# V-Sense/LFBM5D

Hardware: AMD Instinct MI355X
Metric: SAI-megapixels/sec (HT+Wiener, sigma=25) (higher is better)
Workload: dtype f32; 1 GPU; lf17x17x512x512_sigma25; light_field=17x17x512x512x3, asw=1, color_space=opp, noise=MT19937 seed 1 (utilities.cpp:176-183), window_lanes=2, spatial_bands=1, parallelism=single GPU

## Files before the change

### lfbm5d_amd/core.py

```python
import ctypes as C
import os
import subprocess

from typing import NamedTuple, Optional

import numpy as np

_HERE = os.path.dirname(os.path.abspath(__file__))

YUV, YCBCR, OPP, RGB, ID, DCT, SADCT, BIOR, HADAMARD, HAAR = range(10)
ROWMAJOR, COLMAJOR = 11, 12
TAU = {"id": ID, "dct": DCT, "sadct": SADCT, "bior": BIOR, "hw": HADAMARD, "haar": HAAR}
COLOR_SPACE = {"yuv": YUV, "ycbcr": YCBCR, "opp": OPP, "rgb": RGB}
UNIQUE_ID_BYTES = 128


class LfBm5dError(RuntimeError):
    pass


class Params(C.Structure):
    _fields_ = [("sigma", C.c_float), ("lambda_", C.c_float), ("N", C.c_uint), ("nSim", C.c_uint),
                ("nDisp", C.c_uint), ("k", C.c_uint), ("p", C.c_uint), ("useSD", C.c_uint),
                ("tau_2D", C.c_uint), ("tau_4D", C.c_uint), ("tau_5D", C.c_uint),
# ... 194 lines not shown
    dp = C.POINTER(C.c_double)
    if lib().lfbm5d_noise_level_statistic(d, cov.ctypes.data_as(dp), C.byref(sig), C.byref(m), lam.ctypes.data_as(dp)) != 0:
        raise LfBm5dError("lfbm5d_noise_level_statistic: bad arguments (d must be 1..64)")
    return sig.value, m.value, lam


def shard_rows(n_rows, rank, world):
    b, e = C.c_uint(), C.c_uint()
    lib().lfbm5d_shard_rows(n_rows, rank, world, C.byref(b), C.byref(e))
    return b.value, e.value


def make_params(sigma, lam, N, nSim, nDisp, k, p, tau_2D, tau_4D, tau_5D, useSD=0, color_space=OPP):
    t = lambda v: TAU[v] if isinstance(v, str) else int(v)
    cs = COLOR_SPACE[color_space] if isinstance(color_space, str) else int(color_space)
    return Params(float(sigma), float(lam), int(N), int(nSim), int(nDisp), int(k), int(p),
                  int(bool(useSD)), t(tau_2D), t(tau_4D), t(tau_5D), cs)


def make_bm3d_params(sigma, lam, N, nHW, k, p, tau_2D, useSD=0, color_space=OPP):
    cs = COLOR_SPACE[color_space] if isinstance(color_space, str) else int(color_space)
    return Bm3dParams(float(sigma), float(lam), int(N), int(nHW), int(k), int(p), int(bool(useSD)),
                      TAU[tau_2D] if isinstance(tau_2D, str) else int(tau_2D), cs)


def _u32(a):
    return np.ascontiguousarray(np.asarray(a, dtype=np.uint32))


def _dev_ptr(t):
    import torch
    if not (isinstance(t, torch.Tensor) and t.is_cuda and t.dtype == torch.float32 and t.is_contiguous()):
        raise LfBm5dError("device entry points need contiguous float32 CUDA tensors")
    torch.cuda.current_stream(t.device).synchronize()
    return C.c_void_p(t.data_ptr())


def _sai_ptrs(arrays, mask):
    out = (C.c_void_p * len(arrays))()
    for i, a in enumerate(arrays):
        if a is None or not mask[i]:
            continue
        if not (isinstance(a, np.ndarray) and a.dtype == np.float32 and a.flags.c_contiguous):
            raise LfBm5dError("per-SAI host buffers must be contiguous float32 numpy arrays")
        out[i] = a.ctypes.data
    return out


OPTION_ENV = ("LFBM5D_LANES", "LFBM5D_EMULATE_WORLD", "LFBM5D_MAX_WINDOWS", "LFBM5D_FUSED", "LFBM5D_STEP_SHARDING",
              "LFBM5D_DATA_DRIVEN_SCHEDULE", "LFBM5D_HOST_BLOCKING", "LFBM5D_BAND_MB", "LFBM5D_BM3D_LANES", "LFBM5D_SCAN_LDS_CAP",
              "LFBM5D_FORCE_REDO", "LFBM5D_SPATIAL_BANDS", "LFBM5D_BAND_HALO", "LFBM5D_SCAN_V1", "LFBM5D_SCAN_ANY", "LFBM5D_SCAN_FULL_TABLES", "LFBM5D_DCT8W_V2",
              "LFBM5D_GROUP_GENERIC", "LFBM5D_NO_SA_KERNELS", "LFBM5D_NO_SLAB_KERNEL", "LFBM5D_WIDE_NOSPLIT", "LFBM5D_AGG_64BIT",
              "LFBM5D_AGG_SCALAR_SCAN", "LFBM5D_SUBSET_LIST_HOST", "LFBM5D_SUBSET_SCAN_V1", "LFBM5D_FILT_GROUP_MAJOR",
              "LFBM5D_HT_REF_ORDER")


class Context:

    def __init__(self, device=0):
        self._L = lib()
        h = C.c_void_p()
        if self._L.lfbm5d_create(C.byref(h), int(device)) != 0:
            raise LfBm5dError(self._L.lfbm5d_last_error(None).decode())
        self._handle = h
        self._env_seen = {k: os.environ.get(k) for k in OPTION_ENV}
        self.device = int(device)

    @property
    def _h(self):
        h = self._handle
        if h and hasattr(self._L, "lfbm5d_set_option"):
            for k in OPTION_ENV:
                v = os.environ.get(k)
                if v != self._env_seen[k]:
                    self._env_seen[k] = v
                    self._L.lfbm5d_set_option(h, k.encode(), None if v is None else (v or "1").encode())
        return h

    def set_option(self, key, value):
        if self._L.lfbm5d_set_option(self._handle, key.encode(), None if value is None else str(value).encode()) != 0:
            raise LfBm5dError(self._L.lfbm5d_last_error(self._handle).decode())

    def get_option(self, key):
        buf = C.create_string_buffer(64)
        if self._L.lfbm5d_get_option(self._handle, key.encode(), buf, 64) != 0:
            raise LfBm5dError(self._L.lfbm5d_last_error(self._handle).decode())
        return buf.value.decode()

    def close(self):
        if getattr(self, "_handle", None):
            self._L.lfbm5d_destroy(self._handle)
            self._handle = None

    def __del__(self):
        try:
            self.close()
        except Exception:
            pass

    def _ck(self, rc):
        if rc != 0:
            raise LfBm5dError(self._L.lfbm5d_last_error(self._h).decode())

    @staticmethod
    def unique_id():
        buf = (C.c_ubyte * UNIQUE_ID_BYTES)()
        if lib().lfbm5d_comm_unique_id(buf) != 0:
# ... 237 lines not shown
```

### lfbm5d_amd/csrc/lfbm5d_group_wiener.hip

```cpp
#include "lfbm5d_group_device.h"

namespace lfbm5d {

namespace {

constexpr int kDct8Threads = 320;

__global__ __launch_bounds__(kDct8Threads) void k_group_dct8(GroupArgs a) {
    extern __shared__ float lds[];
    __shared__ unsigned pos[kMaxN * kA3];
    __shared__ float red[3][kDct8Threads / 64];
    const int tid = threadIdx.x;
    const unsigned g = a.ref_begin + blockIdx.x;
    const int c = blockIdx.y;
    constexpr int A = 9, K2 = 64;
    const int N = a.N;
    const int nSx = (int)a.self_cnt[g];
    const size_t plane = (size_t)a.Wb * a.Hb;
    const int NP = nSx * A;
    const int NPp = (N * A) | 1;
    float* S0 = lds;
    float* S1 = lds + K2 * NPp;
    const TbPtr tb = (TbPtr)a.tb;

// ... 719 lines not shown
            const float Nn = (float)(nSx * A);
            const float res = (q - m * m / Nn) / (Nn - 1.0f);
            wx = res > 0.0f ? 1.0f / sqrtf(res) : 0.0f;
        } else {
            const float sig = a.sigma[c];
            wx = w > 0.0f ? (sig > 0.0f ? 1.0f / (sig * sig * w) : 1.0f / w) : 1.0f;
        }
        a.wgt[(size_t)g * a.C + c] = wx;
        if (c == 0) {
            atomicAdd(&a.counters[0], (unsigned long long)nSx);
            if (use_sadct) atomicAdd(&a.counters[1], 1ull);
        }
    }

    PHASE_MARK();
    const int NPh = (NP + 1) / 2;
    for (int it = tid; it < NPh * 8; it += TH) {
        const int j = (int)__umulhi((unsigned)it, rcpNPh), pa = it - j * NPh;
        const int pb = pa + NPh < NP ? pa + NPh : pa;
        float* ca = stackf + 2 * (j * NPp + pa) + 1;
        float* cb = stackf + 2 * (j * NPp + pb) + 1;
        v2f x[8];
#pragma unroll
        for (int i = 0; i < 8; i++) x[i] = v2f{ca[2 * (i * 8) * NPp], cb[2 * (i * 8) * NPp]};
        dct8_inv_t(x);
#pragma unroll
        for (int i = 0; i < 8; i++) { ca[2 * (i * 8) * NPp] = x[i].x; if (pb != pa) cb[2 * (i * 8) * NPp] = x[i].y; }
    }
    __syncthreads();
    PHASE_MARK();
    for (int it = tid; it < NP * 8; it += TH) {
        const int patch = it >> 3, i = it & 7;
        const float* ra = stackf + 2 * ((i * 8) * NPp + patch) + 1;
        float x[8];
#pragma unroll
        for (int j = 0; j < 8; j++) x[j] = ra[2 * j * NPp];
        dct8_inv_t(x);
        float4* oa = reinterpret_cast<float4*>(a.filt + ((size_t)g * N * A + patch) * a.C * K2 + (size_t)c * K2 + i * 8);
        filt_put4(&oa[0], make_float4(x[0], x[1], x[2], x[3]));
        filt_put4(&oa[1], make_float4(x[4], x[5], x[6], x[7]));
    }
#ifdef LFBM5D_PHASE_TIMING
    PHASE_MARK();
    if (tid == 0) {
        for (int i = 0; i < 5; i++) atomicAdd(&a.counters[4 + i], (unsigned long long)(tc[i + 1] - tc[i]));
        atomicAdd(&a.counters[9], 1ull);
    }
#endif
}

constexpr int kDct8w3Threads = 256;
constexpr int kW3Stride = 146;
constexpr unsigned kW3Lds = 64 * kW3Stride * sizeof(float);
constexpr unsigned kW3Empty = 0xf0000000u;

template <int NS, int TH> struct W3Rows {
    static constexpr int kIt = (((NS * 9 + 1) / 2) * 8 + TH - 1) / TH;
    v4f ra0[kIt], ra1[kIt], rb0[kIt], rb1[kIt];
};
template <int NS, int TH>
__device__ __forceinline__ void w3_load_rows(__amdgpu_buffer_rsrc_t img, unsigned row_bytes, const unsigned* pos, int tid, W3Rows<NS, TH>& r) {
    constexpr int A = 9, NP = NS * A, NPh = (NP + 1) / 2;
#pragma unroll
    for (int q = 0; q < W3Rows<NS, TH>::kIt; q++) {
        const int it = tid + q * TH;
        if (it < NPh * 8) {
            const int i = it / NPh, pp = it - i * NPh;
            const int pA = 2 * pp, pB = pA + 1 < NP ? pA + 1 : pA;
            const int oa = (int)(pos[pA] + (unsigned)i * row_bytes), ob = (int)(pos[pB] + (unsigned)i * row_bytes);
            r.ra0[q] = __builtin_bit_cast(v4f, __builtin_amdgcn_raw_buffer_load_b128(img, oa, 0, 0));
            r.ra1[q] = __builtin_bit_cast(v4f, __builtin_amdgcn_raw_buffer_load_b128(img, oa + 16, 0, 0));
            r.rb0[q] = __builtin_bit_cast(v4f, __builtin_amdgcn_raw_buffer_load_b128(img, ob, 0, 0));
            r.rb1[q] = __builtin_bit_cast(v4f, __builtin_amdgcn_raw_buffer_load_b128(img, ob + 16, 0, 0));
        }
    }
}
template <int NS, int TH, bool SA, bool U = false>
__device__ __forceinline__ void w3_forward(__amdgpu_buffer_rsrc_t img, unsigned row_bytes, float* S, const unsigned* pos,
                                           int tid, ShRef sh, bool do_dct4, bool do_sa4, TbPtr tb, const W3Rows<NS, TH>* pre = nullptr) {
    constexpr int A = 9, NP = NS * A, NPh = (NP + 1) / 2, NPf = kW3Stride;
    constexpr int kIt = (NPh * 8 + TH - 1) / TH;
    {
        W3Rows<NS, TH> own;
        if (!pre) w3_load_rows<NS, TH>(img, row_bytes, pos, tid, own);
        const W3Rows<NS, TH>& R = pre ? *pre : own;
        const v4f (&ra0)[kIt] = R.ra0; const v4f (&ra1)[kIt] = R.ra1; const v4f (&rb0)[kIt] = R.rb0; const v4f (&rb1)[kIt] = R.rb1;
#pragma unroll
        for (int q = 0; q < kIt; q++) {
            const int it = tid + q * TH;
            if (it < NPh * 8) {
                const int i = it / NPh, pp = it - i * NPh;
                v2f x[8];
#pragma unroll
                for (int j = 0; j < 4; j++) {
                    x[j] = v2f{ra0[q][j], rb0[q][j]};
                    x[4 + j] = v2f{ra1[q][j], rb1[q][j]};
                }
                dct8_fwd_t(x);
                float* dst = S + (i * 8) * NPf + 2 * pp;
#pragma unroll
                for (int j = 0; j < 8; j++) *reinterpret_cast<v2f*>(dst + j * NPf) = x[j];
            }
        }
    }
    __syncthreads();
    for (int it = tid; it < NPh * 8; it += TH) {
        const int j = it / NPh, pp = it - j * NPh;
        float* col = S + j * NPf + 2 * pp;
        v2f x[8];
#pragma unroll
        for (int i = 0; i < 8; i++) x[i] = *reinterpret_cast<const v2f*>(col + (i * 8) * NPf);
        dct8_fwd_t(x);
#pragma unroll
        for (int i = 0; i < 8; i++) *reinterpret_cast<v2f*>(col + (i * 8) * NPf) = x[i];
    }
    __syncthreads();
    if (do_dct4 || do_sa4) {
        for (int f = tid; f < NS * 32; f += TH) {
            int n, pq;
            if (NS > 1) { pq = (f & 15) | ((f >> 1) & 16); n = ((f >> 4) & 1) | ((f >> 5) & ~1); }
            else { n = 0; pq = f; }
            float* b0 = S + pq * NPf + n * A;
            float* b1 = b0 + 32 * NPf;
            v2f x[9];
#pragma unroll
            for (int st = 0; st < 9; st++) x[st] = v2f{b0[st], b1[st]};
            if (U) dct9_fwd2_u(x);
            else if (do_dct4) dct9_fwd2_fast(x, tb);
            else {
                float t9[9];
#pragma unroll
                for (int i = 0; i < 9; i++) t9[i] = x[i].x;
                if (SA) sadct9_fwd_sel(t9, sh, tb); else sadct9_fwd(t9, sh, tb);
#pragma unroll
                for (int i = 0; i < 9; i++) { x[i].x = t9[i]; t9[i] = x[i].y; }
                if (SA) sadct9_fwd_sel(t9, sh, tb); else sadct9_fwd(t9, sh, tb);
#pragma unroll
                for (int i = 0; i < 9; i++) x[i].y = t9[i];
            }
#pragma unroll
            for (int st = 0; st < 9; st++) { b0[st] = x[st].x; b1[st] = x[st].y; }
        }
        __syncthreads();
    }
}

template <int NS, int TH, bool SA>
__device__ __forceinline__ void w3_body(const GroupArgs& a, float* S, const unsigned* pos, float (*red)[TH / 64], int tid,
                                        unsigned g, int c) {
    constexpr int A = 9, K2 = 64, NP = NS * A, NPh = (NP + 1) / 2, NPf = kW3Stride;
    static_assert(TH == 256, "the fibre phases deal st 0..3 / 4..7 to 256 threads");
    const int N = a.N;
    const unsigned win_bytes = (unsigned)((size_t)A * a.C * a.Wb * a.Hb * 4);
    const TbPtr tb = (TbPtr)a.tb;
    ShRef sh = group_shape(a, g);
    const bool use_sadct = a.tau4 == 6 && sh.use_sadct;
    const bool do_dct4 = a.tau4 == 5 || (a.tau4 == 6 && !use_sadct);
    const bool do_sa4 = !do_dct4 && a.tau4 == 6;
    const float sig = a.sigma[c];
    const float sig2 = sig * sig;
    const bool useSD = a.useSD != 0;

    w3_forward<NS, TH, SA>(__builtin_amdgcn_make_buffer_rsrc((void*)a.basic, 0, (int)win_bytes, 0x00020000u), a.Wb * 4u, S, pos, tid, sh, do_dct4, do_sa4, tb);
    const int fpq = (tid & 15) | ((tid >> 1) & 48), fst = ((tid >> 4) & 1) | ((tid >> 6) & 2);
    float* const fbase = S + fpq * NPf + fst;
    float* const f8base = S + (tid & 63) * NPf + 8;
    const bool own8 = tid < 64;
    v2f vv[NS];
    float v8[NS];
    {
        v2f e[NS];
// ... 102 lines not shown
            }
#pragma unroll
            for (int st = 0; st < 9; st++) { b0[st] = x[st].x; b1[st] = x[st].y; }
        }
    }
    __syncthreads();
    if (tid == 0) {
        float w = 0.0f, m = 0.0f, q = 0.0f;
        for (int i = 0; i < TH / 64; i++) { w += red[0][i]; m += red[1][i]; q += red[2][i]; }
        float wx;
        if (a.useSD) {
            const float Nn = (float)(NS * A);
            const float res = (q - m * m / Nn) / (Nn - 1.0f);
            wx = res > 0.0f ? 1.0f / sqrtf(res) : 0.0f;
        } else {
            wx = w > 0.0f ? (sig > 0.0f ? 1.0f / (sig * sig * w) : 1.0f / w) : 1.0f;
        }
        a.wgt[(size_t)g * a.C + c] = wx;
        if (c == 0) {
            atomicAdd(&a.counters[0], (unsigned long long)NS);
            if (use_sadct) atomicAdd(&a.counters[1], 1ull);
        }
    }
    for (int it = tid; it < NPh * 8; it += TH) {
        const int j = it / NPh, pp = it - j * NPh;
        float* col = S + j * NPf + 2 * pp;
        v2f x[8];
#pragma unroll
        for (int i = 0; i < 8; i++) x[i] = *reinterpret_cast<const v2f*>(col + (i * 8) * NPf);
        dct8_inv_t(x);
#pragma unroll
        for (int i = 0; i < 8; i++) *reinterpret_cast<v2f*>(col + (i * 8) * NPf) = x[i];
    }
    __syncthreads();
    for (int it = tid; it < NPh * 8; it += TH) {
        const int pa = it >> 3, i = it & 7;
        const bool has_b = pa + NPh < NP;
        const float* ra = S + (i * 8) * NPf + pa;
        v2f x[8];
#pragma unroll
        for (int j = 0; j < 8; j++) x[j] = v2f{ra[j * NPf], ra[j * NPf + (NP > NPh ? NPh : 0)]};
        dct8_inv_t(x);
        v4f* oa = reinterpret_cast<v4f*>(a.filt + ((size_t)g * N * A + pa) * a.C * K2 + (size_t)c * K2 + i * 8);
        filt_put4_nt(oa, v4f{x[0].x, x[1].x, x[2].x, x[3].x});
        filt_put4_nt(oa + 1, v4f{x[4].x, x[5].x, x[6].x, x[7].x});
        if (has_b) {
            v4f* ob = oa + (size_t)NPh * a.C * (K2 / 4);
            filt_put4_nt(ob, v4f{x[0].y, x[1].y, x[2].y, x[3].y});
            filt_put4_nt(ob + 1, v4f{x[4].y, x[5].y, x[6].y, x[7].y});
        }
    }
}

template <int NS, int TH>
__device__ __forceinline__ void w3_body_u(const GroupArgs& a, float* S, const unsigned* pos, float (*red)[TH / 64], int tid, unsigned g, int c) {
    constexpr int A = 9, K2 = 64, NP = NS * A, NPh = (NP + 1) / 2, NPf = kW3Stride;
    constexpr int L = NS == 16 ? 4 : NS == 8 ? 3 : NS == 4 ? 2 : NS == 2 ? 1 : 0;
    static_assert(TH == 256, "the fibre phases deal st 0..3 / 4..7 to 256 threads");
    const int N = a.N;
    const unsigned win_bytes = (unsigned)((size_t)A * a.C * a.Wb * a.Hb * 4);
    const TbPtr tb = (TbPtr)a.tb;
    ShRef sh = group_shape(a, g);
    const float sig = a.sigma[c];
    const float sig2 = sig * sig;
    const bool useSD = a.useSD != 0;

    w3_forward<NS, TH, false, true>(__builtin_amdgcn_make_buffer_rsrc((void*)a.basic, 0, (int)win_bytes, 0x00020000u), a.Wb * 4u, S, pos, tid, sh, true, false, tb);
    const int fpq = (tid & 15) | ((tid >> 1) & 48), fst = ((tid >> 4) & 1) | ((tid >> 6) & 2);
    float* const fbase = S + fpq * NPf + fst;
    float* const f8base = S + (tid & 63) * NPf + 8;
    const bool own8 = tid < 64;
    v2f kq[L + 1];
    float k8[L + 1];
    {
        const float fa = tb->ht3_f[fst], fb = tb->ht3_f[fst + 4], f8 = tb->ht3_f[8];
        const v2f q = v2f{sig2 / (fa * fa), sig2 / (fb * fb)};
        const float q8 = sig2 / (f8 * f8);
#pragma unroll
        for (int l = 0; l <= L; l++) { kq[l] = q * (float)(1 << l); k8[l] = q8 * (float)(1 << l); }
    }
    v2f vv[NS];
    float v8[NS];
    {
        v2f e[NS];
#pragma unroll
        for (int n = 0; n < NS; n++) e[n] = v2f{fbase[n * A], fbase[n * A + 4]};
        haar_fwd_u<NS>(e);
#pragma unroll
        for (int n = 0; n < NS; n++) {
            const v2f value = e[n] * e[n], den = value + kq[haar_level<NS>(n)];
            vv[n] = v2f{wiener_div(value.x, den.x), wiener_div(value.y, den.y)};
        }
    }
    if (own8) {
        float e[NS];
#pragma unroll
        for (int n = 0; n < NS; n++) e[n] = f8base[n * A];
        haar_fwd_u<NS>(e);
#pragma unroll
        for (int n = 0; n < NS; n++) {
            const float value = e[n] * e[n];
            v8[n] = wiener_div(value, value + k8[haar_level<NS>(n)]);
        }
    }
    __syncthreads();
    w3_forward<NS, TH, false, true>(__builtin_amdgcn_make_buffer_rsrc((void*)a.noisy, 0, (int)win_bytes, 0x00020000u), a.Wb * 4u, S, pos, tid, sh, true, false, tb);
    float wacc = 0.0f, s1 = 0.0f, s2 = 0.0f;
    const float inv_n = 1.0f / (float)NS;
    {
        v2f o[NS];
#pragma unroll
        for (int n = 0; n < NS; n++) o[n] = v2f{fbase[n * A], fbase[n * A + 4]};
        haar_fwd_u<NS>(o);
        v2f w2 = v2f{0.f, 0.f};
#pragma unroll
        for (int n = 0; n < NS; n++) { o[n] = o[n] * vv[n]; w2 += vv[n]; }
        wacc = w2.x + w2.y;
        haar_inv_u<NS>(o);
#pragma unroll
        for (int n = 0; n < NS; n++) { fbase[n * A] = o[n].x; fbase[n * A + 4] = o[n].y; }
        if (useSD) {
            const v2f f2 = v2f{tb->ht3_f[fst], tb->ht3_f[fst + 4]} * inv_n;
#pragma unroll
            for (int n = 0; n < NS; n++) { const v2f y = o[n] * f2; s1 += y.x + y.y; s2 += y.x * y.x + y.y * y.y; }
        }
    }
    if (own8) {
        float o[NS];
#pragma unroll
        for (int n = 0; n < NS; n++) o[n] = f8base[n * A];
        haar_fwd_u<NS>(o);
#pragma unroll
        for (int n = 0; n < NS; n++) { o[n] = o[n] * v8[n]; wacc += v8[n]; }
        haar_inv_u<NS>(o);
#pragma unroll
        for (int n = 0; n < NS; n++) f8base[n * A] = o[n];
        if (useSD) {
            const float f2 = tb->ht3_f[8] * inv_n;
#pragma unroll
            for (int n = 0; n < NS; n++) { const float y = o[n] * f2; s1 += y; s2 += y * y; }
        }
    }
    for (int o = 32; o > 0; o >>= 1) { wacc += __shfl_xor(wacc, o); s1 += __shfl_xor(s1, o); s2 += __shfl_xor(s2, o); }
    if ((tid & 63) == 0) { red[0][tid >> 6] = wacc; red[1][tid >> 6] = s1; red[2][tid >> 6] = s2; }
    __syncthreads();
    for (int f = tid; f < NS * 32; f += TH) {
        int n, pq;
        if (NS > 1) { pq = (f & 15) | ((f >> 1) & 16); n = ((f >> 4) & 1) | ((f >> 5) & ~1); }
        else { n = 0; pq = f; }
        float* b0 = S + pq * NPf + n * A;
        float* b1 = b0 + 32 * NPf;
        v2f x[9];
#pragma unroll
        for (int st = 0; st < 9; st++) x[st] = v2f{b0[st], b1[st]};
        dct9_inv2_u(x, tb, inv_n);
#pragma unroll
        for (int st = 0; st < 9; st++) { b0[st] = x[st].x; b1[st] = x[st].y; }
    }
    __syncthreads();
    if (tid == 0) {
        float w = 0.0f, m = 0.0f, q = 0.0f;
        for (int i = 0; i < TH / 64; i++) { w += red[0][i]; m += red[1][i]; q += red[2][i]; }
        float wx;
        if (a.useSD) {
            const float Nn = (float)(NS * A);
            const float res = (q - m * m / Nn) / (Nn - 1.0f);
            wx = res > 0.0f ? 1.0f / sqrtf(res) : 0.0f;
        } else {
            wx = w > 0.0f ? (sig > 0.0f ? 1.0f / (sig * sig * w) : 1.0f / w) : 1.0f;
        }
        a.wgt[(size_t)g * a.C + c] = wx;
        if (c == 0) atomicAdd(&a.counters[0], (unsigned long long)NS);
    }
    for (int it = tid; it < NPh * 8; it += TH) {
        const int j = it / NPh, pp = it - j * NPh;
        float* col = S + j * NPf + 2 * pp;
        v2f x[8];
#pragma unroll
        for (int i = 0; i < 8; i++) x[i] = *reinterpret_cast<const v2f*>(col + (i * 8) * NPf);
        dct8_inv_t(x);
#pragma unroll
        for (int i = 0; i < 8; i++) *reinterpret_cast<v2f*>(col + (i * 8) * NPf) = x[i];
    }
    __syncthreads();
    for (int it = tid; it < NPh * 8; it += TH) {
        const int pa = it >> 3, i = it & 7;
        const bool has_b = pa + NPh < NP;
        const float* ra = S + (i * 8) * NPf + pa;
        v2f x[8];
#pragma unroll
        for (int j = 0; j < 8; j++) x[j] = v2f{ra[j * NPf], ra[j * NPf + (NP > NPh ? NPh : 0)]};
        dct8_inv_t(x);
        v4f* oa = reinterpret_cast<v4f*>(a.filt + ((size_t)g * N * A + pa) * a.C * K2 + (size_t)c * K2 + i * 8);
        filt_put4_nt(oa, v4f{x[0].x, x[1].x, x[2].x, x[3].x});
        filt_put4_nt(oa + 1, v4f{x[4].x, x[5].x, x[6].x, x[7].x});
        if (has_b) {
            v4f* ob = oa + (size_t)NPh * a.C * (K2 / 4);
            filt_put4_nt(ob, v4f{x[0].y, x[1].y, x[2].y, x[3].y});
            filt_put4_nt(ob + 1, v4f{x[4].y, x[5].y, x[6].y, x[7].y});
        }
    }
}

constexpr int kW3SaWaves = 4;
template <bool SA>
__global__ __launch_bounds__(kDct8w3Threads) __attribute__((amdgpu_waves_per_eu(SA ? kW3SaWaves : 1))) void k_group_dct8w3(GroupArgs a) {
    extern __shared__ float lds[];
    __shared__ float red[3][kDct8w3Threads / 64];
    __shared__ unsigned pos[kMaxN * kA3];
    constexpr int TH = kDct8w3Threads;
    const int tid = threadIdx.x;
    const unsigned gi = xcd_group_index(a);
    if (gi >= a.n_groups) return;
    const unsigned g = a.ref_begin + gi;
    const int c = blockIdx.y;
    const int nSx = (int)a.self_cnt[g];
    const unsigned plane = a.Wb * a.Hb;
    for (int i = tid; i < nSx * 9; i += TH) {
        const unsigned p = a.gpos[(size_t)g * a.N * 9 + i];
        pos[i] = p != 0xffffffffu ? (((unsigned)(i % 9) * a.C + c) * plane + p) * 4u : kW3Empty;
    }
    __syncthreads();
    switch (nSx) {
        case 1:  w3_body<1, TH, SA>(a, lds, pos, red, tid, g, c); break;
        case 2:  w3_body<2, TH, SA>(a, lds, pos, red, tid, g, c); break;
        case 4:  w3_body<4, TH, SA>(a, lds, pos, red, tid, g, c); break;
        case 8:  w3_body<8, TH, SA>(a, lds, pos, red, tid, g, c); break;
        default: w3_body<16, TH, SA>(a, lds, pos, red, tid, g, c); break;
    }
}

__global__ __launch_bounds__(kDct8w3Threads) void k_group_dct8w3_u(GroupArgs a) {
    extern __shared__ float lds[];
    __shared__ float red[3][kDct8w3Threads / 64];
    __shared__ unsigned pos[kMaxN * kA3];
    constexpr int TH = kDct8w3Threads;
    const int tid = threadIdx.x;
    const unsigned gi = xcd_group_index(a);
    if (gi >= a.n_groups) return;
    const unsigned g = a.ref_begin + gi;
    if (a.tau4 == 6 && group_shape(a, g).use_sadct) return;
    const int c = blockIdx.y;
    const int nSx = (int)a.self_cnt[g];
    const unsigned plane = a.Wb * a.Hb;
    for (int i = tid; i < nSx * 9; i += TH) {
        const unsigned p = a.gpos[(size_t)g * a.N * 9 + i];
        pos[i] = p != 0xffffffffu ? (((unsigned)(i % 9) * a.C + c) * plane + p) * 4u : kW3Empty;
    }
    __syncthreads();
    switch (nSx) {
        case 1:  w3_body_u<1, TH>(a, lds, pos, red, tid, g, c); break;
        case 2:  w3_body_u<2, TH>(a, lds, pos, red, tid, g, c); break;
        case 4:  w3_body_u<4, TH>(a, lds, pos, red, tid, g, c); break;
        case 8:  w3_body_u<8, TH>(a, lds, pos, red, tid, g, c); break;
        default: w3_body_u<16, TH>(a, lds, pos, red, tid, g, c); break;
    }
}
constexpr unsigned kW3ListBlocks = 256;
__global__ __launch_bounds__(kDct8w3Threads) void k_group_dct8w3_list(GroupArgs a) {
    extern __shared__ float lds[];
    __shared__ float red[3][kDct8w3Threads / 64];
    __shared__ unsigned pos[kMaxN * kA3];
    constexpr int TH = kDct8w3Threads;
    const int tid = threadIdx.x;
    const unsigned n_list = a.sa_list[0];
    const int c = blockIdx.y;
    for (unsigned li = blockIdx.x; li < n_list; li += gridDim.x) {
        const unsigned g = a.sa_list[1u + li] & 0x1fffffffu;
        const int nSx = (int)a.self_cnt[g];
        const unsigned plane = a.Wb * a.Hb;
        for (int i = tid; i < nSx * 9; i += TH) {
            const unsigned p = a.gpos[(size_t)g * a.N * 9 + i];
            pos[i] = p != 0xffffffffu ? (((unsigned)(i % 9) * a.C + c) * plane + p) * 4u : kW3Empty;
        }
        __syncthreads();
        switch (nSx) {
            case 1:  w3_body<1, TH, true>(a, lds, pos, red, tid, g, c); break;
            case 2:  w3_body<2, TH, true>(a, lds, pos, red, tid, g, c); break;
            case 4:  w3_body<4, TH, true>(a, lds, pos, red, tid, g, c); break;
            case 8:  w3_body<8, TH, true>(a, lds, pos, red, tid, g, c); break;
            default: w3_body<16, TH, true>(a, lds, pos, red, tid, g, c); break;
        }
        __syncthreads();
    }
}

constexpr int kBm3dWaves = 4;
template <int STEP> struct Bm3dT { typedef float type; };
template <> struct Bm3dT<2> { typedef v2f type; };
__device__ __forceinline__ float bm3d_first(float x) { return x; }
__device__ __forceinline__ float bm3d_first(v2f x) { return x.x; }

template <int STEP, bool BIOR>
__global__ __launch_bounds__(64 * kBm3dWaves) void k_group_bm3d8(GroupArgs a) {
    extern __shared__ float lds[];
    typedef typename Bm3dT<STEP>::type T;
    constexpr int K2 = 64, ST = kMaxN3 + 1;
    const int wave = threadIdx.x >> 6, lane = threadIdx.x & 63;
    const unsigned gi = blockIdx.x * kBm3dWaves + wave;
    if (gi >= a.n_groups) return;
    const unsigned g = a.ref_begin + gi;
    const int c = blockIdx.y;
    const int N = a.N, nSx = (int)a.self_cnt[g];
    const size_t plane = (size_t)a.Wb * a.Hb;
    const TbPtr tb = (TbPtr)a.tb;
    T* S = reinterpret_cast<T*>(lds) + (size_t)wave * K2 * ST;

    if (lane < nSx) {
// ... 94 lines not shown
        else {
#pragma unroll
            for (int j = 0; j < 8; j++) {
                float col[8];
#pragma unroll
                for (int i = 0; i < 8; i++) col[i] = x[i][j];
                dct8_inv_t(col);
#pragma unroll
                for (int i = 0; i < 8; i++) x[i][j] = col[i];
            }
#pragma unroll
            for (int i = 0; i < 8; i++) dct8_inv_t(x[i]);
        }
        float4* dst = reinterpret_cast<float4*>(a.filt + (((size_t)g * N + lane) * a.C + c) * K2);
#pragma unroll
        for (int i = 0; i < 8; i++) {
            filt_put4(&dst[2 * i], make_float4(x[i][0], x[i][1], x[i][2], x[i][3]));
            filt_put4(&dst[2 * i + 1], make_float4(x[i][4], x[i][5], x[i][6], x[i][7]));
        }
    }
}

}

hipError_t prepare_group_wiener() {
    const void* fns[] = {
        reinterpret_cast<const void*>(&k_group_dct8),
        reinterpret_cast<const void*>(&k_group_dct8w2<true>), reinterpret_cast<const void*>(&k_group_dct8w2<false>),
        reinterpret_cast<const void*>(&k_group_dct8w<true>), reinterpret_cast<const void*>(&k_group_dct8w<false>),
        reinterpret_cast<const void*>(&k_group_bm3d8<2, true>), reinterpret_cast<const void*>(&k_group_bm3d8<2, false>)};
    for (const void* f : fns) {
        const hipError_t e = hipFuncSetAttribute(f, hipFuncAttributeMaxDynamicSharedMemorySize, kDedicatedLdsLimit);
        if (e != hipSuccess) return e;
    }
    return hipSuccess;
}

hipError_t launch_group_wiener(hipStream_t s, const GroupArgs& a, bool all_sa, bool* launched) {
    *launched = true;
    if (a.tau2 == 7 && a.k == 8 && a.A == 9 && a.step == 2 && a.N <= (unsigned)kMaxN) {
        const size_t l8 = (size_t)2 * 64 * ((a.N * 9) | 1) * sizeof(float);
        if (a.tau5 == 9) hipLaunchKernelGGL((k_group_dct8w<true>), dim3(a.n_groups, a.C), dim3(kDct8wThreads), l8, s, a);
        else             hipLaunchKernelGGL((k_group_dct8w<false>), dim3(a.n_groups, a.C), dim3(kDct8wThreads), l8, s, a);
        return hipGetLastError();
    }
    if (a.tau2 == 5 && a.k == 8 && a.A == 9 && a.N <= (unsigned)kMaxN) {
        const size_t l8 = (size_t)(a.step == 2 ? 2 : 1) * 64 * ((a.N * 9) | 1) * sizeof(float);
        if (a.step == 2) {
            const unsigned gx = ((a.n_groups + 7) / 8) * 8;
            if (a.tau5 == 9 && (size_t)9 * a.C * a.Wb * a.Hb * 4 < 0x70000000ull && !(a.opt & kOptDct8wV2)) {
                if (all_sa) hipLaunchKernelGGL(k_group_dct8w3<true>, dim3(gx, a.C), dim3(kDct8w3Threads), kW3Lds, s, a);
                else if (a.tau4 == 5 || a.tau4 == 6) {
                    if (!a.sa_list) return hipErrorInvalidValue;
                    hipLaunchKernelGGL(k_group_dct8w3_u, dim3(gx, a.C), dim3(kDct8w3Threads), kW3Lds, s, a);
                    if (a.tau4 == 6) hipLaunchKernelGGL(k_group_dct8w3_list, dim3(kW3ListBlocks, a.C), dim3(kDct8w3Threads), kW3Lds, s, a);
                }
                else        hipLaunchKernelGGL(k_group_dct8w3<false>, dim3(gx, a.C), dim3(kDct8w3Threads), kW3Lds, s, a);
            }
            else if (a.tau5 == 9) hipLaunchKernelGGL((k_group_dct8w2<true>), dim3(gx, a.C), dim3(kDct8w2Threads), l8, s, a);
            else                  hipLaunchKernelGGL((k_group_dct8w2<false>), dim3(gx, a.C), dim3(kDct8w2Threads), l8, s, a);
            return hipGetLastError();
        }
        hipLaunchKernelGGL(k_group_dct8, dim3(a.n_groups, a.C), dim3(kDct8Threads), l8, s, a);
        return hipGetLastError();
    }
    if (a.bm3d && a.A == 1 && a.k == 8 && a.tau5 == 8 && (a.tau2 == 5 || a.tau2 == 7)) {
        const dim3 grid((a.n_groups + kBm3dWaves - 1) / kBm3dWaves, a.C), block(64 * kBm3dWaves);
        const size_t lb = (size_t)kBm3dWaves * 64 * (kMaxN3 + 1) * (a.step == 2 ? sizeof(v2f) : sizeof(float));
        if (a.step == 2) { if (a.tau2 == 7) hipLaunchKernelGGL((k_group_bm3d8<2, true>), grid, block, lb, s, a); else hipLaunchKernelGGL((k_group_bm3d8<2, false>), grid, block, lb, s, a); }
        else             { if (a.tau2 == 7) hipLaunchKernelGGL((k_group_bm3d8<1, true>), grid, block, lb, s, a); else hipLaunchKernelGGL((k_group_bm3d8<1, false>), grid, block, lb, s, a); }
        return hipGetLastError();
    }
    *launched = false;
    return hipSuccess;
}
}
```

### lfbm5d_amd/csrc/lfbm5d_options.h

```cpp
#ifndef LFBM5D_OPTIONS_H
#define LFBM5D_OPTIONS_H

#include <cstddef>
#include <cstdlib>
#include <cstring>
#include <string>

namespace lfbm5d {

enum : unsigned {
    kOptScanV1 = 1u << 0,
    kOptScanAny = 1u << 1,
    kOptScanFullTables = 1u << 2,
    kOptDct8wV2 = 1u << 3,
    kOptGroupGeneric = 1u << 4,
    kOptNoSaKernels = 1u << 5,
    kOptNoSlabKernel = 1u << 6,
    kOptWideNoSplit = 1u << 7,
    kOptAgg64Bit = 1u << 8,
    kOptAggScalarScan = 1u << 9,
    kOptSubsetListHost = 1u << 10,
    kOptSubsetScanV1 = 1u << 11,
    kOptFiltGroupMajor = 1u << 12,
    kOptHtReferenceOrder = 1u << 13,
};

struct Options {
    int lanes = 2;
    int emulate_world = 0;
    int max_windows = 0;
    int fused = 1;
    int step_sharding = 0;
    int data_driven_schedule = 0;
    int host_blocking = 0;
    int band_mb = 0;
    int bm3d_lanes = 3;
    int scan_lds_cap = 0;
    int force_redo = 0;
    int spatial_bands = 1;
    int band_halo = 0;
    unsigned kernels = 0;
};

struct OptionKey { const char* key; const char* env; int Options::* field; unsigned bit; };

inline const OptionKey* option_keys(size_t* n) {
    static const OptionKey keys[] = {
        {"lanes", "LFBM5D_LANES", &Options::lanes, 0}, {"emulate_world", "LFBM5D_EMULATE_WORLD", &Options::emulate_world, 0},
        {"max_windows", "LFBM5D_MAX_WINDOWS", &Options::max_windows, 0}, {"fused", "LFBM5D_FUSED", &Options::fused, 0},
        {"step_sharding", "LFBM5D_STEP_SHARDING", &Options::step_sharding, 0},
        {"data_driven_schedule", "LFBM5D_DATA_DRIVEN_SCHEDULE", &Options::data_driven_schedule, 0},
        {"host_blocking", "LFBM5D_HOST_BLOCKING", &Options::host_blocking, 0}, {"band_mb", "LFBM5D_BAND_MB", &Options::band_mb, 0},
        {"bm3d_lanes", "LFBM5D_BM3D_LANES", &Options::bm3d_lanes, 0}, {"scan_lds_cap", "LFBM5D_SCAN_LDS_CAP", &Options::scan_lds_cap, 0},
        {"force_redo", "LFBM5D_FORCE_REDO", &Options::force_redo, 0}, {"spatial_bands", "LFBM5D_SPATIAL_BANDS", &Options::spatial_bands, 0},
        {"band_halo", "LFBM5D_BAND_HALO", &Options::band_halo, 0},
        {"scan_v1", "LFBM5D_SCAN_V1", nullptr, kOptScanV1}, {"scan_any", "LFBM5D_SCAN_ANY", nullptr, kOptScanAny},
        {"scan_full_tables", "LFBM5D_SCAN_FULL_TABLES", nullptr, kOptScanFullTables}, {"dct8w_v2", "LFBM5D_DCT8W_V2", nullptr, kOptDct8wV2},
        {"group_generic", "LFBM5D_GROUP_GENERIC", nullptr, kOptGroupGeneric}, {"no_sa_kernels", "LFBM5D_NO_SA_KERNELS", nullptr, kOptNoSaKernels},
        {"no_slab_kernel", "LFBM5D_NO_SLAB_KERNEL", nullptr, kOptNoSlabKernel}, {"wide_nosplit", "LFBM5D_WIDE_NOSPLIT", nullptr, kOptWideNoSplit},
        {"agg_64bit", "LFBM5D_AGG_64BIT", nullptr, kOptAgg64Bit}, {"agg_scalar_scan", "LFBM5D_AGG_SCALAR_SCAN", nullptr, kOptAggScalarScan},
        {"subset_list_host", "LFBM5D_SUBSET_LIST_HOST", nullptr, kOptSubsetListHost}, {"subset_scan_v1", "LFBM5D_SUBSET_SCAN_V1", nullptr, kOptSubsetScanV1},
        {"filt_group_major", "LFBM5D_FILT_GROUP_MAJOR", nullptr, kOptFiltGroupMajor},
        {"ht_reference_order", "LFBM5D_HT_REF_ORDER", nullptr, kOptHtReferenceOrder},
    };
    *n = sizeof(keys) / sizeof(keys[0]);
    return keys;
}

inline bool option_set(Options& o, const char* key, const char* value) {
    size_t n; const OptionKey* keys = option_keys(&n);
    static const Options defaults;
    for (size_t i = 0; i < n; i++) {
        if (std::strcmp(key, keys[i].key) != 0 && std::strcmp(key, keys[i].env) != 0) continue;
        const bool unset = value == nullptr || value[0] == 0;
        if (keys[i].field) {
            int v = defaults.*(keys[i].field);
            if (!unset) {
                if (keys[i].field == &Options::step_sharding) v = std::strcmp(value, "rows") == 0 ? 1 : std::strcmp(value, "blocks") == 0 ? 2 : std::atoi(value);
                else if (keys[i].field == &Options::data_driven_schedule || keys[i].field == &Options::host_blocking || keys[i].field == &Options::force_redo)
                    v = std::strcmp(value, "0") != 0;
                else v = std::atoi(value);
            }
            o.*(keys[i].field) = v;
        } else {
            if (!unset && std::strcmp(value, "0") != 0) o.kernels |= keys[i].bit; else o.kernels &= ~keys[i].bit;
        }
        return true;
    }
    return false;
}
inline bool option_get(const Options& o, const char* key, std::string& out) {
    size_t n; const OptionKey* keys = option_keys(&n);
    for (size_t i = 0; i < n; i++) {
        if (std::strcmp(key, keys[i].key) != 0 && std::strcmp(key, keys[i].env) != 0) continue;
        if (keys[i].field == &Options::step_sharding) out = o.step_sharding == 1 ? "rows" : o.step_sharding == 2 ? "blocks" : "0";
        else if (keys[i].field) out = std::to_string(o.*(keys[i].field));
        else out = (o.kernels & keys[i].bit) ? "1" : "0";
        return true;
    }
    return false;
}
inline void options_from_env(Options& o) {
    size_t n; const OptionKey* keys = option_keys(&n);
    for (size_t i = 0; i < n; i++)
        if (const char* e = std::getenv(keys[i].env)) {
            const bool flag = !keys[i].field || keys[i].field == &Options::data_driven_schedule || keys[i].field == &Options::host_blocking ||
                              keys[i].field == &Options::force_redo;
            if (e[0]) (void)option_set(o, keys[i].key, e); else if (flag) (void)option_set(o, keys[i].key, "1");
        }
}

}
#endif
```

Measured before the change: 243.7 SAI-megapixels/s.

## Keep Wiener 4D/5D fibre transforms in registers with a banded LDS layout for 16-match groups

Adds a register-resident fibre stage for the 16-match unstructured Wiener group kernel. Patches are loaded in a permuted order into a padded banded LDS layout, so each thread owns a 4-wide fibre slab and does the DCT9 plus Haar-like match transform with DPP quad exchanges, instead of the previous multi-pass LDS fibre phases. It also rotates thread-to-work assignment per block to spread LDS bank and memory access patterns, and sets waves_per_eu to 4 for the new path. The old LDS fibre path stays behind a new option. The new path is the default, and it risks higher register pressure and possible differences in rounding from the fused/unfused denominators.

```diff
diff --git a/lfbm5d_amd/core.py b/lfbm5d_amd/core.py
--- a/lfbm5d_amd/core.py
+++ b/lfbm5d_amd/core.py
@@ -270,7 +270,7 @@
               "LFBM5D_FORCE_REDO", "LFBM5D_SPATIAL_BANDS", "LFBM5D_BAND_HALO", "LFBM5D_SCAN_V1", "LFBM5D_SCAN_ANY", "LFBM5D_SCAN_FULL_TABLES", "LFBM5D_DCT8W_V2",
               "LFBM5D_GROUP_GENERIC", "LFBM5D_NO_SA_KERNELS", "LFBM5D_NO_SLAB_KERNEL", "LFBM5D_WIDE_NOSPLIT", "LFBM5D_AGG_64BIT",
               "LFBM5D_AGG_SCALAR_SCAN", "LFBM5D_SUBSET_LIST_HOST", "LFBM5D_SUBSET_SCAN_V1", "LFBM5D_FILT_GROUP_MAJOR",
-              "LFBM5D_HT_REF_ORDER")
+              "LFBM5D_HT_REF_ORDER", "LFBM5D_W3_LDS_FIBRES")
 
 
 class Context:
diff --git a/lfbm5d_amd/csrc/lfbm5d_group_wiener.hip b/lfbm5d_amd/csrc/lfbm5d_group_wiener.hip
--- a/lfbm5d_amd/csrc/lfbm5d_group_wiener.hip
+++ b/lfbm5d_amd/csrc/lfbm5d_group_wiener.hip
@@ -795,13 +795,25 @@
 constexpr int kDct8w3Threads = 256;
 constexpr int kW3Stride = 146;
 constexpr unsigned kW3Lds = 64 * kW3Stride * sizeof(float);
+constexpr int kW3StrideF = 144, kW3BandF = 8 * kW3StrideF + 4;
+__device__ __forceinline__ int w3_patch_of(int col) {
+    const int qq = col / 36, rem = col - 36 * qq;
+    return (4 * qq + (rem & 3)) * 9 + (rem >> 2);
+}
+static_assert((7 * kW3BandF + 8 * kW3StrideF) * sizeof(float) <= kW3Lds, "the fibre layout fits the stack of the previous one");
+template <bool F> struct W3Lay {
+    static constexpr int kStride = F ? kW3StrideF : kW3Stride, kBand = F ? kW3BandF : 8 * kW3Stride;
+};
+constexpr bool kW3Rotate = true;
+__device__ __forceinline__ int w3_rot0() { return kW3Rotate ? (int)(blockIdx.x + (blockIdx.x >> 8) + blockIdx.y) : 0; }
+template <int TH> __device__ __forceinline__ int w3_rot_tid(int tid, int rot) { return kW3Rotate ? (tid + 64 * rot) & (TH - 1) : tid; }
 constexpr unsigned kW3Empty = 0xf0000000u;
 
 template <int NS, int TH> struct W3Rows {
     static constexpr int kIt = (((NS * 9 + 1) / 2) * 8 + TH - 1) / TH;
     v4f ra0[kIt], ra1[kIt], rb0[kIt], rb1[kIt];
 };
-template <int NS, int TH>
+template <int NS, int TH, bool F = false>
 __device__ __forceinline__ void w3_load_rows(__amdgpu_buffer_rsrc_t img, unsigned row_bytes, const unsigned* pos, int tid, W3Rows<NS, TH>& r) {
     constexpr int A = 9, NP = NS * A, NPh = (NP + 1) / 2;
 #pragma unroll
@@ -809,7 +821,7 @@
         const int it = tid + q * TH;
         if (it < NPh * 8) {
             const int i = it / NPh, pp = it - i * NPh;
-            const int pA = 2 * pp, pB = pA + 1 < NP ? pA + 1 : pA;
+            const int pA = F ? w3_patch_of(2 * pp) : 2 * pp, pB = F ? pA + A : pA + 1 < NP ? pA + 1 : pA;
             const int oa = (int)(pos[pA] + (unsigned)i * row_bytes), ob = (int)(pos[pB] + (unsigned)i * row_bytes);
             r.ra0[q] = __builtin_bit_cast(v4f, __builtin_amdgcn_raw_buffer_load_b128(img, oa, 0, 0));
             r.ra1[q] = __builtin_bit_cast(v4f, __builtin_amdgcn_raw_buffer_load_b128(img, oa + 16, 0, 0));
@@ -818,14 +830,16 @@
         }
     }
 }
-template <int NS, int TH, bool SA, bool U = false>
+template <int NS, int TH, bool SA, bool U = false, bool F = false, bool ROT = false>
 __device__ __forceinline__ void w3_forward(__amdgpu_buffer_rsrc_t img, unsigned row_bytes, float* S, const unsigned* pos,
-                                           int tid, ShRef sh, bool do_dct4, bool do_sa4, TbPtr tb, const W3Rows<NS, TH>* pre = nullptr) {
-    constexpr int A = 9, NP = NS * A, NPh = (NP + 1) / 2, NPf = kW3Stride;
+                                           int tid, ShRef sh, bool do_dct4, bool do_sa4, TbPtr tb, const W3Rows<NS, TH>* pre = nullptr, int rot = 0) {
+    constexpr int A = 9, NP = NS * A, NPh = (NP + 1) / 2, NPf = W3Lay<F>::kStride, NB = W3Lay<F>::kBand;
     constexpr int kIt = (NPh * 8 + TH - 1) / TH;
+    const int ftid = tid;
+    if (ROT) tid = w3_rot_tid<TH>(tid, rot);
     {
         W3Rows<NS, TH> own;
-        if (!pre) w3_load_rows<NS, TH>(img, row_bytes, pos, tid, own);
+        if (!pre) w3_load_rows<NS, TH, F>(img, row_bytes, pos, tid, own);
         const W3Rows<NS, TH>& R = pre ? *pre : own;
         const v4f (&ra0)[kIt] = R.ra0; const v4f (&ra1)[kIt] = R.ra1; const v4f (&rb0)[kIt] = R.rb0; const v4f (&rb1)[kIt] = R.rb1;
 #pragma unroll
@@ -840,26 +854,27 @@
                     x[4 + j] = v2f{ra1[q][j], rb1[q][j]};
                 }
                 dct8_fwd_t(x);
-                float* dst = S + (i * 8) * NPf + 2 * pp;
+                float* dst = S + i * NB + 2 * pp;
 #pragma unroll
                 for (int j = 0; j < 8; j++) *reinterpret_cast<v2f*>(dst + j * NPf) = x[j];
             }
         }
     }
     __syncthreads();
+    if (ROT) tid = w3_rot_tid<TH>(tid, 1);
     for (int it = tid; it < NPh * 8; it += TH) {
         const int j = it / NPh, pp = it - j * NPh;
         float* col = S + j * NPf + 2 * pp;
         v2f x[8];
 #pragma unroll
-        for (int i = 0; i < 8; i++) x[i] = *reinterpret_cast<const v2f*>(col + (i * 8) * NPf);
+        for (int i = 0; i < 8; i++) x[i] = *reinterpret_cast<const v2f*>(col + i * NB);
         dct8_fwd_t(x);
 #pragma unroll
-        for (int i = 0; i < 8; i++) *reinterpret_cast<v2f*>(col + (i * 8) * NPf) = x[i];
-    }
-    __syncthreads();
-    if (do_dct4 || do_sa4) {
-        for (int f = tid; f < NS * 32; f += TH) {
+        for (int i = 0; i < 8; i++) *reinterpret_cast<v2f*>(col + i * NB) = x[i];
+    }
+    __syncthreads();
+    if (!F && (do_dct4 || do_sa4)) {
+        for (int f = ftid; f < NS * 32; f += TH) {
             int n, pq;
             if (NS > 1) { pq = (f & 15) | ((f >> 1) & 16); n = ((f >> 4) & 1) | ((f >> 5) & ~1); }
             else { n = 0; pq = f; }
@@ -1068,11 +1083,120 @@
     }
 }
 
-template <int NS, int TH>
+template <int CTRL> __device__ __forceinline__ float w3_quad(float v) {
+    return __builtin_bit_cast(float, __builtin_amdgcn_mov_dpp(__builtin_bit_cast(int, v), CTRL, 0xf, 0xf, false));
+}
+__device__ __forceinline__ float w3_flip(float v, unsigned sign) { return __builtin_bit_cast(float, __builtin_bit_cast(unsigned, v) ^ sign); }
+__device__ __forceinline__ float w3_den(float e, float k, bool fused) {
+#pragma clang fp contract(off)
+    const float value = e * e;
+    return fused ? __builtin_fmaf(e, e, k) : value + k;
+}
+struct W3Fibres {
+    float* fb;
+    const bool odd;
+    const unsigned m_odd, m_hi;
+    TbPtr tb;
+    float kq[9];
+    v2f c1[9];
+    float c2[9], cq[9];
+
+    __device__ __forceinline__ W3Fibres(float* S, int tid, float sig2, TbPtr t)
+        : fb(S + (tid >> 5) * kW3BandF + ((tid >> 2) & 7) * kW3StrideF + 36 * (tid & 3)), odd(tid & 1), m_odd((unsigned)(tid & 1) << 31),
+          m_hi((unsigned)(tid & 2) << 30), tb(t) {
+#pragma unroll
+        for (int st = 0; st < 9; st++) {
+            const float f = tb->ht3_f[st];
+            kq[st] = __builtin_bit_cast(float, __builtin_amdgcn_readfirstlane(__builtin_bit_cast(int, sig2 / (f * f))));
+        }
+    }
+    __device__ __forceinline__ void forward(v2f* d1, float* d2, float* dq) const {
+        v4f r[9];
+#pragma unroll
+        for (int k = 0; k < 9; k++) r[k] = *reinterpret_cast<const v4f*>(fb + 4 * k);
+        v2f xa[9], xb[9];
+#pragma unroll
+        for (int st = 0; st < 9; st++) { xa[st] = v2f{r[st][0], r[st][1]}; xb[st] = v2f{r[st][2], r[st][3]}; }
+        dct9_fwd2_u(xa);
+        __builtin_amdgcn_sched_barrier(0);
+        dct9_fwd2_u(xb);
+        __builtin_amdgcn_sched_barrier(0);
+#pragma unroll
+        for (int st = 0; st < 9; st++) {
+            const v2f s = v2f{xa[st].x + xa[st].y, xb[st].x + xb[st].y};
+            d1[st] = v2f{xa[st].x - xa[st].y, xb[st].x - xb[st].y};
+            const float a2 = s.x + s.y;
+            d2[st] = s.x - s.y;
+            const float r3 = w3_quad<0xB1>(a2) + w3_flip(a2, m_odd);
+            const float r4 = w3_quad<0x4E>(r3) + w3_flip(r3, m_hi);
+            dq[st] = odd ? r3 : r4;
+        }
+    }
+    __device__ __forceinline__ float pilot() {
+        v2f d1[9];
+        float d2[9], dq[9];
+        forward(d1, d2, dq);
+        float w = 0.0f;
+#pragma unroll
+        for (int st = 0; st < 9; st++) {
+            const float k = kq[st];
+            const float den1x = w3_den(d1[st].x, 2.0f * k, st < 8), den1y = w3_den(d1[st].y, 2.0f * k, st < 8);
+            const float den2 = w3_den(d2[st], 4.0f * k, st < 8), denq = w3_den(dq[st], (odd ? 8.0f : 16.0f) * k, false);
+            c1[st] = v2f{wiener_div(d1[st].x * d1[st].x, den1x), wiener_div(d1[st].y * d1[st].y, den1y)};
+            c2[st] = wiener_div(d2[st] * d2[st], den2);
+            cq[st] = wiener_div(dq[st] * dq[st], denq);
+        }
+#pragma unroll
+        for (int st = 0; st < 9; st++) {
+            asm volatile("" : "+v"(c1[st].x), "+v"(c1[st].y), "+v"(c2[st]), "+v"(cq[st]));
+            w += (c1[st].x + c1[st].y) + (c2[st] + cq[st]);
+        }
+        asm volatile("" : "+v"(w));
+        return w;
+    }
+    __device__ __forceinline__ void noisy(bool useSD, float inv_n, float& s1, float& s2) const {
+        v2f xa[9], xb[9];
+        {
+            v2f d1[9];
+            float d2[9], dq[9];
+            forward(d1, d2, dq);
+            const float w2 = odd ? -2.0f : 2.0f;
+#pragma unroll
+            for (int st = 0; st < 9; st++) {
+                const v2f e1 = d1[st] * c1[st];
+                const float e2 = d2[st] * c2[st], eq = dq[st] * cq[st];
+                const float b1 = w3_quad<0x00>(eq) + w3_flip(w3_quad<0xAA>(eq), m_hi);
+                const float b2 = __builtin_fmaf(w3_quad<0xF5>(eq), w2, b1);
+                const v2f a1 = v2f{__builtin_fmaf(4.0f, e2, b2), __builtin_fmaf(-4.0f, e2, b2)};
+                xa[st] = v2f{__builtin_fmaf(8.0f, e1.x, a1.x), __builtin_fmaf(-8.0f, e1.x, a1.x)};
+                xb[st] = v2f{__builtin_fmaf(8.0f, e1.y, a1.y), __builtin_fmaf(-8.0f, e1.y, a1.y)};
+            }
+        }
+        if (useSD) {
+#pragma unroll
+            for (int st = 0; st < 9; st++) {
+                const float f2 = tb->ht3_f[st] * inv_n;
+                const float o[4] = {xa[st].x, xa[st].y, xb[st].x, xb[st].y};
+#pragma unroll
+                for (int m = 0; m < 4; m++) { const float y = o[m] * f2; s1 += y; s2 += y * y; }
+            }
+        }
+        __builtin_amdgcn_sched_barrier(0);
+        dct9_inv2_u(xa, tb, inv_n);
+        __builtin_amdgcn_sched_barrier(0);
+        dct9_inv2_u(xb, tb, inv_n);
+#pragma unroll
+        for (int st = 0; st < 9; st++) *reinterpret_cast<v4f*>(fb + 4 * st) = v4f{xa[st].x, xa[st].y, xb[st].x, xb[st].y};
+    }
+};
+
+template <int NS, int TH, bool F = false>
 __device__ __forceinline__ void w3_body_u(const GroupArgs& a, float* S, const unsigned* pos, float (*red)[TH / 64], int tid, unsigned g, int c) {
-    constexpr int A = 9, K2 = 64, NP = NS * A, NPh = (NP + 1) / 2, NPf = kW3Stride;
+    constexpr int A = 9, K2 = 64, NP = NS * A, NPh = (NP + 1) / 2, NPf = W3Lay<F>::kStride, NB = W3Lay<F>::kBand;
     constexpr int L = NS == 16 ? 4 : NS == 8 ? 3 : NS == 4 ? 2 : NS == 2 ? 1 : 0;
-    static_assert(TH == 256, "the fibre phases deal st 0..3 / 4..7 to 256 threads");
+    static_assert(TH == 256, "the fibre phases deal st 0..3 / 4..7 (F: the four quarters of a fibre) to 256 threads");
+    static_assert(!F || NS == 16, "the register-resident fibre stage is written for 16 matches");
+    const int rot = w3_rot0();
     const int N = a.N;
     const unsigned win_bytes = (unsigned)((size_t)A * a.C * a.Wb * a.Hb * 4);
     const TbPtr tb = (TbPtr)a.tb;
@@ -1081,7 +1205,19 @@
     const float sig2 = sig * sig;
     const bool useSD = a.useSD != 0;
 
-    w3_forward<NS, TH, false, true>(__builtin_amdgcn_make_buffer_rsrc((void*)a.basic, 0, (int)win_bytes, 0x00020000u), a.Wb * 4u, S, pos, tid, sh, true, false, tb);
+    w3_forward<NS, TH, false, true, F, kW3Rotate>(__builtin_amdgcn_make_buffer_rsrc((void*)a.basic, 0, (int)win_bytes, 0x00020000u), a.Wb * 4u, S, pos, tid, sh, true, false, tb, nullptr, rot);
+    float wacc = 0.0f, s1 = 0.0f, s2 = 0.0f;
+    const float inv_n = 1.0f / (float)NS;
+    if constexpr (F) {
+    W3Fibres fib(S, tid, sig2, tb);
+    wacc = fib.pilot();
+    __syncthreads();
+    w3_forward<NS, TH, false, true, true, kW3Rotate>(__builtin_amdgcn_make_buffer_rsrc((void*)a.noisy, 0, (int)win_bytes, 0x00020000u), a.Wb * 4u, S, pos, tid, sh, true, false, tb, nullptr, rot + 2);
+    fib.noisy(useSD, inv_n, s1, s2);
+    for (int o = 32; o > 0; o >>= 1) { wacc += __shfl_xor(wacc, o); s1 += __shfl_xor(s1, o); s2 += __shfl_xor(s2, o); }
+    if ((tid & 63) == 0) { red[0][tid >> 6] = wacc; red[1][tid >> 6] = s1; red[2][tid >> 6] = s2; }
+    __syncthreads();
+    } else {
     const int fpq = (tid & 15) | ((tid >> 1) & 48), fst = ((tid >> 4) & 1) | ((tid >> 6) & 2);
     float* const fbase = S + fpq * NPf + fst;
     float* const f8base = S + (tid & 63) * NPf + 8;
@@ -1120,9 +1256,7 @@
         }
     }
     __syncthreads();
-    w3_forward<NS, TH, false, true>(__builtin_amdgcn_make_buffer_rsrc((void*)a.noisy, 0, (int)win_bytes, 0x00020000u), a.Wb * 4u, S, pos, tid, sh, true, false, tb);
-    float wacc = 0.0f, s1 = 0.0f, s2 = 0.0f;
-    const float inv_n = 1.0f / (float)NS;
+    w3_forward<NS, TH, false, true, false, kW3Rotate>(__builtin_amdgcn_make_buffer_rsrc((void*)a.noisy, 0, (int)win_bytes, 0x00020000u), a.Wb * 4u, S, pos, tid, sh, true, false, tb, nullptr, rot + 2);
     {
         v2f o[NS];
 #pragma unroll
@@ -1174,6 +1308,7 @@
         for (int st = 0; st < 9; st++) { b0[st] = x[st].x; b1[st] = x[st].y; }
     }
     __syncthreads();
+    }
     if (tid == 0) {
         float w = 0.0f, m = 0.0f, q = 0.0f;
         for (int i = 0; i < TH / 64; i++) { w += red[0][i]; m += red[1][i]; q += red[2][i]; }
@@ -1188,21 +1323,21 @@
         a.wgt[(size_t)g * a.C + c] = wx;
         if (c == 0) atomicAdd(&a.counters[0], (unsigned long long)NS);
     }
-    for (int it = tid; it < NPh * 8; it += TH) {
+    for (int it = w3_rot_tid<TH>(tid, rot + 4); it < NPh * 8; it += TH) {
         const int j = it / NPh, pp = it - j * NPh;
         float* col = S + j * NPf + 2 * pp;
         v2f x[8];
 #pragma unroll
-        for (int i = 0; i < 8; i++) x[i] = *reinterpret_cast<const v2f*>(col + (i * 8) * NPf);
+        for (int i = 0; i < 8; i++) x[i] = *reinterpret_cast<const v2f*>(col + i * NB);
         dct8_inv_t(x);
 #pragma unroll
-        for (int i = 0; i < 8; i++) *reinterpret_cast<v2f*>(col + (i * 8) * NPf) = x[i];
-    }
-    __syncthreads();
-    for (int it = tid; it < NPh * 8; it += TH) {
-        const int pa = it >> 3, i = it & 7;
+        for (int i = 0; i < 8; i++) *reinterpret_cast<v2f*>(col + i * NB) = x[i];
+    }
+    __syncthreads();
+    for (int it = w3_rot_tid<TH>(tid, rot + 5); it < NPh * 8; it += TH) {
+        const int pcol = it >> 3, i = it & 7, pa = F ? w3_patch_of(pcol) : pcol;
         const bool has_b = pa + NPh < NP;
-        const float* ra = S + (i * 8) * NPf + pa;
+        const float* ra = S + i * NB + pcol;
         v2f x[8];
 #pragma unroll
         for (int j = 0; j < 8; j++) x[j] = v2f{ra[j * NPf], ra[j * NPf + (NP > NPh ? NPh : 0)]};
@@ -1246,7 +1381,8 @@
     }
 }
 
-__global__ __launch_bounds__(kDct8w3Threads) void k_group_dct8w3_u(GroupArgs a) {
+template <bool F>
+__global__ __launch_bounds__(kDct8w3Threads) __attribute__((amdgpu_waves_per_eu(F ? 4 : 1))) void k_group_dct8w3_u(GroupArgs a) {
     extern __shared__ float lds[];
     __shared__ float red[3][kDct8w3Threads / 64];
     __shared__ unsigned pos[kMaxN * kA3];
@@ -1269,7 +1405,7 @@
         case 2:  w3_body_u<2, TH>(a, lds, pos, red, tid, g, c); break;
         case 4:  w3_body_u<4, TH>(a, lds, pos, red, tid, g, c); break;
         case 8:  w3_body_u<8, TH>(a, lds, pos, red, tid, g, c); break;
-        default: w3_body_u<16, TH>(a, lds, pos, red, tid, g, c); break;
+        default: w3_body_u<16, TH, F>(a, lds, pos, red, tid, g, c); break;
     }
 }
 constexpr unsigned kW3ListBlocks = 256;
@@ -1470,7 +1606,8 @@
                 if (all_sa) hipLaunchKernelGGL(k_group_dct8w3<true>, dim3(gx, a.C), dim3(kDct8w3Threads), kW3Lds, s, a);
                 else if (a.tau4 == 5 || a.tau4 == 6) {
                     if (!a.sa_list) return hipErrorInvalidValue;
-                    hipLaunchKernelGGL(k_group_dct8w3_u, dim3(gx, a.C), dim3(kDct8w3Threads), kW3Lds, s, a);
+                    if (a.opt & kOptW3LdsFibres) hipLaunchKernelGGL(k_group_dct8w3_u<false>, dim3(gx, a.C), dim3(kDct8w3Threads), kW3Lds, s, a);
+                    else                         hipLaunchKernelGGL(k_group_dct8w3_u<true>, dim3(gx, a.C), dim3(kDct8w3Threads), kW3Lds, s, a);
                     if (a.tau4 == 6) hipLaunchKernelGGL(k_group_dct8w3_list, dim3(kW3ListBlocks, a.C), dim3(kDct8w3Threads), kW3Lds, s, a);
                 }
                 else        hipLaunchKernelGGL(k_group_dct8w3<false>, dim3(gx, a.C), dim3(kDct8w3Threads), kW3Lds, s, a);
diff --git a/lfbm5d_amd/csrc/lfbm5d_options.h b/lfbm5d_amd/csrc/lfbm5d_options.h
--- a/lfbm5d_amd/csrc/lfbm5d_options.h
+++ b/lfbm5d_amd/csrc/lfbm5d_options.h
@@ -23,6 +23,7 @@
     kOptSubsetScanV1 = 1u << 11,
     kOptFiltGroupMajor = 1u << 12,
     kOptHtReferenceOrder = 1u << 13,
+    kOptW3LdsFibres = 1u << 14,
 };
 
 struct Options {
@@ -62,6 +63,7 @@
         {"subset_list_host", "LFBM5D_SUBSET_LIST_HOST", nullptr, kOptSubsetListHost}, {"subset_scan_v1", "LFBM5D_SUBSET_SCAN_V1", nullptr, kOptSubsetScanV1},
         {"filt_group_major", "LFBM5D_FILT_GROUP_MAJOR", nullptr, kOptFiltGroupMajor},
         {"ht_reference_order", "LFBM5D_HT_REF_ORDER", nullptr, kOptHtReferenceOrder},
+        {"w3_lds_fibres", "LFBM5D_W3_LDS_FIBRES", nullptr, kOptW3LdsFibres},
     };
     *n = sizeof(keys) / sizeof(keys[0]);
     return keys;
```

Result: no change. 242.7 SAI-megapixels/s (-0.4%).
